# LongmaoTeamTf/deep_recommenders

Measured on AMD Instinct MI355X. Metric: examples/sec/node DeepFM (26 sparse feats, 10M vocab, dim 64), higher is better.
Workload: dtype f32; 1 GPU; DeepFM Criteo-shape synthetic training step (BASELINE.json configs[2]): 26 sparse + 13 dense, 10000000 vocab/field hashed on device, dim 64, DNN [256, 32]+[1] relu, sigmoid-CE, fused SGD; batch 65536 per GPU, ids uniform; tables on one GPU (66.6 GB); gemm_split=f16x2, global_batch=65536, parallelism=single, per_kernel_events=False

## Files before the change

deep_recommenders_amd/csrc/h2_occ.hip:

```cpp
#include "dr_common.h"
#include "rs_args.h"
#include <cstdlib>

namespace drrs {
namespace {

typedef _Float16 f16x4 __attribute__((ext_vector_type(4)));
typedef float f32x4 __attribute__((ext_vector_type(4)));
typedef float f32x16 __attribute__((ext_vector_type(16)));
typedef unsigned u32x4 __attribute__((ext_vector_type(4)));
typedef __attribute__((address_space(3))) void* lds_ptr_t;

#define OCC_DS_READ_B128(dst, addr, off) asm volatile("ds_read_b128 %0, %1 offset:%2" : "=v"(dst) : "v"(addr), "n"(off))
#define OCC_DS_WRITE_B64(addr, val, off) asm volatile("ds_write_b64 %0, %1 offset:%2" ::"v"(addr), "v"(val), "n"(off) : "memory")
#define OCC_DS_WRITE_B32(addr, val, off) asm volatile("ds_write_b32 %0, %1 offset:%2" ::"v"(addr), "v"(val), "n"(off) : "memory")

constexpr int BM = 256, BN = 256, BK = 32;
constexpr int PLANE = 256 * 64;
constexpr int A_OFF = 0, B_OFF = 2 * PLANE, STAGE = 4 * PLANE;

struct K4Args {
    const int32_t* ids_t;
    const uint8_t* flags;
    const int64_t* row_base; int32_t F;
    float* table; float* lin_w;
    const float* lin_old_t;
    const float* sum_x; const float* d_fm_logit;
    float scale;
    float* d_concat; int64_t ld_dc;
    uint32_t* table_amax;
};

template <int EPI, int DBG = 0>
__global__ __launch_bounds__(1024) void h2_occ_nt_kernel(RsArgs g, K4Args e) {
    __shared__ __attribute__((aligned(1024))) unsigned char smem[2 * STAGE + (EPI == 8 ? 10240 : 0)];

    const int tid = threadIdx.x, lane = tid & 63;
    const int wave = __builtin_amdgcn_readfirstlane(tid >> 6);
    const int l31 = lane & 31, hi = lane >> 5;
    const int wr = wave >> 2, wc = wave & 3;

    const int tiles_n = (g.N + BN - 1) / BN;
    const int tiles_m = (int)((g.M + BM - 1) / BM);
    const int ntiles = tiles_m * tiles_n;
    const int nk = (g.K + BK - 1) / BK;
    const bool ktail = (g.K % BK) != 0;
    const int kv4 = (g.K + 3) / 4 * 4;

    float s_a, inv_a, s_b, inv_b;
    h2_scale_of(g.a_amax[0], s_a, inv_a);
    h2_scale_of(g.b_amax[0], s_b, inv_b);
    const float h2_out = inv_a * inv_b;
    h2_mode_on();
    float cmax = 0.f;

    const unsigned lds0 = (unsigned)(uintptr_t)(lds_ptr_t)smem;
    const int sw = (l31 >> 2) & 3;
    const unsigned a_rd = lds0 + A_OFF + (64 * wr + l31) * 64 + (((2 * hi) ^ sw) << 4);
    const unsigned b_rd = lds0 + B_OFF + (64 * wc + l31) * 64 + (((2 * hi) ^ sw) << 4);
    const int r8 = lane >> 3, c4 = lane & 7;
    const int arow0 = 16 * wave + r8;
    const unsigned a_wr = lds0 + A_OFF + arow0 * 64 + ((((c4 >> 1) ^ ((arow0 >> 2) & 3)) << 4) | ((c4 & 1) << 3));
    const int avoff0 = (int)((arow0 * g.lda + 4 * c4) * 4), avoff1 = avoff0 + (int)(8 * g.lda * 4);
    const int brow = 16 * wave + (lane >> 2);
    const int bchunk = (lane & 3) ^ ((brow >> 2) & 3);
    const __amdgpu_buffer_rsrc_t brsrc = __builtin_amdgcn_make_buffer_rsrc(
        const_cast<__bf16*>(g.B), 0, (int)min((int64_t)0x7fffffff, 2 * g.b_ps * 2), 0x00020000);
    const int b_plane1 = (int)(g.b_ps * 2);

    f32x16 acc[2][2];
#pragma unroll
    for (int a = 0; a < 2; ++a)
#pragma unroll
        for (int b = 0; b < 2; ++b)
#pragma unroll
            for (int k = 0; k < 16; ++k) acc[a][b][k] = 0.f;

    for (int tile = blockIdx.x; tile < ntiles; tile += gridDim.x) {
        const int lid = xcd_remap(tile, ntiles);
        const int64_t tm0 = (int64_t)(lid / tiles_n) * BM;
        const int tn0 = (lid % tiles_n) * BN;
        const __amdgpu_buffer_rsrc_t arsrc = __builtin_amdgcn_make_buffer_rsrc(
            const_cast<float*>(g.A + tm0 * g.lda), 0, (int)min((int64_t)0x7fffffff, ((g.M - tm0 - 1) * g.lda + kv4) * 4), 0x00020000);
        const int bvoff = (int)(((int64_t)min(tn0 + brow, g.N - 1) * g.b_ld + bchunk * 8) * 2);
        auto issue_b = [&](int kt, int stage) {
            if constexpr (DBG & 1) { if (kt > 0) return; }
#pragma unroll
            for (int p = 0; p < 2; ++p) {
                unsigned char* dst = smem + stage * STAGE + B_OFF + p * PLANE + wave * 1024;
                __builtin_amdgcn_raw_ptr_buffer_load_lds(brsrc, (lds_ptr_t)dst, 16, bvoff, kt * (BK * 2) + p * b_plane1, 0, 0);
            }
        };
        f32x4 an0, an1;
        int an_kt = 0;
        auto load_a = [&](int kt) {
            if constexpr (DBG & 8) kt = 0;
            an_kt = kt;
            an0 = __builtin_bit_cast(f32x4, __builtin_amdgcn_raw_buffer_load_b128(arsrc, avoff0, kt * (BK * 4), 0));
            an1 = __builtin_bit_cast(f32x4, __builtin_amdgcn_raw_buffer_load_b128(arsrc, avoff1, kt * (BK * 4), 0));
        };
        auto wait_a = [&](bool) {};
        auto stage_a = [&](int which, int stage) {
            if constexpr (DBG & 64) return;
            f32x4 v = which == 0 ? an0 : an1;
            if (ktail) {
                const int k = an_kt * BK + 4 * c4;
                v[0] = k < g.K ? v[0] : 0.f; v[1] = k + 1 < g.K ? v[1] : 0.f; v[2] = k + 2 < g.K ? v[2] : 0.f; v[3] = k + 3 < g.K ? v[3] : 0.f;
            }
            f16x4 h, l;
            if constexpr (DBG & 256) {
                typedef float f32x2 __attribute__((ext_vector_type(2)));
                h = __builtin_bit_cast(f16x4, f32x2{v[0], v[1]});
                l = __builtin_bit_cast(f16x4, f32x2{v[2], v[3]});
            } else {
                const f32x4 x = v * s_a;
                h = __builtin_convertvector(x, f16x4);
                l = __builtin_convertvector(x - __builtin_convertvector(h, f32x4), f16x4);
            }
            const unsigned w = (which == 0 ? a_wr : (a_wr ^ 32u) + 512u) + stage * STAGE;
            if constexpr (DBG & 128) {
                asm volatile("" :: "v"(h), "v"(l), "v"(w));
            } else {
                OCC_DS_WRITE_B64(w, h, 0);
                OCC_DS_WRITE_B64(w, l, PLANE);
            }
        };
        f16x8 ah[2], al[2], bh[2], bl[2];
#define OCC_MMA(A, B)                                                                                       \
        _Pragma("unroll") for (int a = 0; a < 2; ++a)                                                       \
            _Pragma("unroll") for (int b = 0; b < 2; ++b)                                                   \
                if constexpr (!(DBG & 2)) acc[a][b] = __builtin_amdgcn_mfma_f32_32x32x16_f16(A[a], B[b], acc[a][b], 0, 0, 0);
#define OCC_MMA2(A, B, AI)                                                                                  \
        _Pragma("unroll") for (int b = 0; b < 2; ++b)                                                       \
            if constexpr (!(DBG & 2)) acc[AI][b] = __builtin_amdgcn_mfma_f32_32x32x16_f16(A[AI], B[b], acc[AI][b], 0, 0, 0);
#define OCC_RD(DST, ADDR, OFF) if constexpr (!(DBG & 32)) OCC_DS_READ_B128(DST, ADDR, OFF); else asm volatile("" : "=v"(DST));
#define OCC_FENCE() __builtin_amdgcn_sched_barrier(0)

        issue_b(0, 0);
        load_a(0);
        OCC_FENCE();
        wait_a(false);
        stage_a(0, 0);
        stage_a(1, 0);
        OCC_FENCE();
        load_a(nk > 1 ? 1 : 0);
        OCC_FENCE();
        asm volatile("s_waitcnt vmcnt(2) lgkmcnt(0)\n\ts_barrier" ::: "memory");
        if (nk > 1) issue_b(1, 1);
        {
            const unsigned aa = a_rd, bb = b_rd;
            OCC_RD(bl[0], bb, PLANE) OCC_RD(bl[1], bb, PLANE + 2048) OCC_RD(al[0], aa, PLANE) OCC_RD(al[1], aa, PLANE + 2048)
            OCC_RD(ah[0], aa, 0) OCC_RD(ah[1], aa, 2048) OCC_RD(bh[0], bb, 0) OCC_RD(bh[1], bb, 2048)
        }
        OCC_FENCE();

        for (int kt = 0; kt < nk; ++kt) {
            const int stage = kt & 1;
            const bool more = kt + 1 < nk;
            const unsigned aa1 = (a_rd + stage * STAGE) ^ 16u, bb1 = (b_rd + stage * STAGE) ^ 16u;
            if constexpr (!(DBG & 32)) asm volatile("s_waitcnt lgkmcnt(2)" : "+v"(ah[0]), "+v"(bl[0]), "+v"(ah[1]), "+v"(bl[1]), "+v"(al[0]), "+v"(al[1]));
            OCC_MMA(ah, bl)
            OCC_FENCE();
            OCC_RD(bl[0], bb1, PLANE) OCC_RD(bl[1], bb1, PLANE + 2048)
            if constexpr (!(DBG & 32)) asm volatile("s_waitcnt lgkmcnt(2)" : "+v"(bh[0]), "+v"(bh[1]));
            OCC_MMA2(al, bh, 0)
            OCC_FENCE();
            if (more) {
                wait_a(true);
                stage_a(0, stage ^ 1);
            }
            OCC_FENCE();
            OCC_MMA2(al, bh, 1)
            OCC_FENCE();
            OCC_RD(al[0], aa1, PLANE) OCC_RD(al[1], aa1, PLANE + 2048)
            OCC_MMA2(ah, bh, 0)
            OCC_FENCE();
            if (more) stage_a(1, stage ^ 1);
            OCC_FENCE();
            OCC_MMA2(ah, bh, 1)
            OCC_FENCE();
            OCC_RD(ah[0], aa1, 0) OCC_RD(ah[1], aa1, 2048) OCC_RD(bh[0], bb1, 0) OCC_RD(bh[1], bb1, 2048)
            load_a(kt + 2 < nk ? kt + 2 : nk - 1);
            OCC_FENCE();
            if constexpr (!(DBG & 32)) asm volatile("s_waitcnt lgkmcnt(2)" : "+v"(ah[0]), "+v"(ah[1]), "+v"(bl[0]), "+v"(bl[1]), "+v"(al[0]), "+v"(al[1]));
            OCC_MMA(ah, bl)
            OCC_FENCE();
            if constexpr (!(DBG & 512)) asm volatile("s_waitcnt vmcnt(2) lgkmcnt(0)\n\ts_barrier" : "+v"(bh[0]), "+v"(bh[1]) :: "memory");
            else asm volatile("s_waitcnt vmcnt(2) lgkmcnt(0)" : "+v"(bh[0]), "+v"(bh[1]) :: "memory");
            if (more) issue_b(kt + 2 < nk ? kt + 2 : nk - 1, stage);
            const unsigned aa2 = a_rd + (stage ^ 1) * STAGE, bb2 = b_rd + (stage ^ 1) * STAGE;
            if (more) { OCC_RD(bl[0], bb2, PLANE) OCC_RD(bl[1], bb2, PLANE + 2048) }
            OCC_FENCE();
            OCC_MMA(al, bh)
            OCC_FENCE();
            if (more) { OCC_RD(al[0], aa2, PLANE) OCC_RD(al[1], aa2, PLANE + 2048) }
            OCC_MMA(ah, bh)
            OCC_FENCE();
            if (more) { OCC_RD(ah[0], aa2, 0) OCC_RD(ah[1], aa2, 2048) OCC_RD(bh[0], bb2, 0) OCC_RD(bh[1], bb2, 2048) }
            OCC_FENCE();
            if constexpr (DBG & 2) acc[0][0][0] += (float)ah[0][0] + (float)ah[1][0] + (float)al[0][0] + (float)al[1][0] + (float)bh[0][0] + (float)bh[1][0] + (float)bl[0][0] + (float)bl[1][0];
        }
#undef OCC_MMA
#undef OCC_MMA2
#undef OCC_RD
#undef OCC_FENCE

        {
            const bool relu = g.act == 1;
            const bool interior = tm0 + BM <= g.M && tn0 + BN <= g.N;
            int lane_e = lane;
            asm volatile("" : "+v"(lane_e));
            const unsigned stg = lds0 + wave * 8192;
            const unsigned st_wr = stg + (4 * (lane_e >> 5)) * 256 + (lane_e & 31) * 4;
            const int prow = lane_e >> 4, pc4 = (lane_e & 15) * 4;
            const unsigned st_rd = stg + prow * 256 + pc4 * 4;
            const int col0 = tn0 + 64 * wc + pc4;
            float4 bj = make_float4(0.f, 0.f, 0.f, 0.f);
            if (g.bias != nullptr) {
                if (interior) bj = *reinterpret_cast<const float4*>(g.bias + col0);
                else {
                    bj.x = g.bias[min(col0, g.N - 1)]; bj.y = g.bias[min(col0 + 1, g.N - 1)];
                    bj.z = g.bias[min(col0 + 2, g.N - 1)]; bj.w = g.bias[min(col0 + 3, g.N - 1)];
                }
            }
            const int k4_f = (tn0 >> 6) + wc;
            const bool k4_on = EPI == 8 && k4_f < e.F;
            const int k4_rows = (int)min((int64_t)BM, g.M - tm0);
            const int k4_ldc4 = (int)(e.ld_dc * 4);
            __amdgpu_buffer_rsrc_t k4_t, k4_dl, k4_lo, k4_sx, k4_dc, k4_lw, k4_id, k4_fl;
            if constexpr (EPI == 8) {
                auto mk = [&](const void* p, int64_t bytes) {
                    const uint64_t b = reinterpret_cast<uint64_t>(p);
                    void* q = reinterpret_cast<void*>(((uint64_t)(unsigned)__builtin_amdgcn_readfirstlane((int)(b >> 32)) << 32) |
                                                      (unsigned)__builtin_amdgcn_readfirstlane((int)b));
                    return __builtin_amdgcn_make_buffer_rsrc(q, 0, (int)(unsigned)(bytes < 0xffffff00ll ? bytes : 0xffffff00ll), 0x00020000);
                };
                const int fc = k4_on ? k4_f : 0;
                const int64_t rb = e.row_base[fc];
                const bool has_lin = e.lin_w != nullptr;
                k4_t = mk(e.table + rb * 64, 0xffffff00ll);
                k4_dl = mk(e.d_fm_logit + tm0, (int64_t)k4_rows * 4);
                k4_lo = has_lin ? mk(e.lin_old_t + (int64_t)fc * g.M + tm0, (int64_t)k4_rows * 4) : k4_dl;
                k4_sx = mk(e.sum_x + tm0 * 64, (int64_t)k4_rows * 256);
                k4_dc = mk(e.d_concat + tm0 * e.ld_dc + 64 * fc, ((int64_t)k4_rows - 1) * e.ld_dc * 4 + 256);
                k4_lw = has_lin ? mk(e.lin_w + rb, 0x7fffffffll) : mk(e.table, 0);
                k4_id = mk(e.ids_t + (int64_t)fc * g.M + tm0, (int64_t)k4_rows * 4);
                k4_fl = mk(e.flags + tm0 * e.F, (int64_t)k4_rows * e.F);
            }
            if constexpr (EPI == 8) {
                constexpr unsigned SXP = 65536, DLP = 2 * STAGE, LOP = 2 * STAGE + 1024, UIP = 2 * STAGE + 1024 + 4096;
                const unsigned stq = lds0 + wave * 4096;
                const unsigned stq_wr = stq + (4 * (lane_e >> 5)) * 256 + (lane_e & 31) * 4;
                const unsigned stq_rd = stq + prow * 256 + pc4 * 4;
                {
#pragma unroll
                    for (int p4 = 0; p4 < 4; ++p4)
                        __builtin_amdgcn_raw_ptr_buffer_load_lds(k4_sx, (lds_ptr_t)(smem + SXP + (16 * wave + 4 * p4) * 256), 16,
                                                                 (16 * wave + 4 * p4 + (lane_e >> 4)) * 256 + (lane_e & 15) * 16, 0, 0, 0);
                    unsigned dlv = __builtin_amdgcn_raw_buffer_load_b32(k4_dl, (64 * wr + lane_e) * 4, 0, 0);
                    unsigned lov = __builtin_amdgcn_raw_buffer_load_b32(k4_lo, (64 * wr + lane_e) * 4, 0, 0);
                    int idl = (int)__builtin_amdgcn_raw_buffer_load_b32(k4_id, (64 * wr + lane_e) * 4, 0, 0);
                    int fll = (int)__builtin_amdgcn_raw_buffer_load_b8(k4_fl, (64 * wr + lane_e) * e.F + k4_f, 0, 0);
                    asm volatile("s_waitcnt vmcnt(0)" : "+v"(dlv), "+v"(lov), "+v"(idl), "+v"(fll) :: "memory");
                    const int uid = (k4_on && 64 * wr + lane_e < k4_rows && idl >= 0 && fll != 0) ? idl : -1;
                    OCC_DS_WRITE_B32(lds0 + DLP + (64 * wr + lane_e) * 4, dlv, 0);
                    OCC_DS_WRITE_B32(lds0 + LOP + wave * 256 + lane_e * 4, lov, 0);
                    OCC_DS_WRITE_B32(lds0 + UIP + wave * 256 + lane_e * 4, uid, 0);
                    asm volatile("s_waitcnt lgkmcnt(0)\n\ts_barrier" ::: "memory");
                }
                if (k4_on) {
#pragma unroll
                    for (int a = 0; a < 2; ++a) {
                        const int ml0 = 64 * wr + 32 * a + prow;
                        unsigned voff[8];
                        unsigned uqm = 0;
                        u32x4 t[8];
#pragma unroll
                        for (int it = 0; it < 8; ++it) {
                            const int uidv = *reinterpret_cast<const int*>(smem + UIP + wave * 256 + (32 * a + 4 * it + prow) * 4);
                            if (uidv >= 0) uqm |= 1u << it;
                            voff[it] = (unsigned)max(uidv, 0) * 256u + (unsigned)pc4 * 4u;
                            t[it] = __builtin_amdgcn_raw_buffer_load_b128(k4_t, (int)voff[it], 0, 2);
                        }
                        asm volatile("s_waitcnt vmcnt(0)" : "+v"(t[0]), "+v"(t[1]), "+v"(t[2]), "+v"(t[3]), "+v"(t[4]), "+v"(t[5]), "+v"(t[6]), "+v"(t[7]));
#pragma unroll
                        for (int q = 0; q < 2; ++q) {
#pragma unroll
                            for (int b = 0; b < 2; ++b)
#pragma unroll
                                for (int r8 = 0; r8 < 8; ++r8) {
                                    const int reg = 8 * q + r8;
                                    const float v = acc[a][b][reg] * h2_out;
                                    acc[a][b][reg] = 0.f;
                                    switch (b * 8 + r8) {
#define OCC_W(I) case I: OCC_DS_WRITE_B32(stq_wr, v, ((I & 3) + 8 * ((I & 7) >> 2)) * 256 + (I >> 3) * 128); break;
                                        OCC_W(0) OCC_W(1) OCC_W(2) OCC_W(3) OCC_W(4) OCC_W(5) OCC_W(6) OCC_W(7) OCC_W(8) OCC_W(9) OCC_W(10) OCC_W(11)
                                        OCC_W(12) OCC_W(13) OCC_W(14) OCC_W(15)
#undef OCC_W
                                    }
                                }
                            f32x4 v[4];
                            asm volatile("s_waitcnt lgkmcnt(0)\n\tds_read_b128 %0, %4 offset:0\n\tds_read_b128 %1, %4 offset:1024\n\t"
                                         "ds_read_b128 %2, %4 offset:2048\n\tds_read_b128 %3, %4 offset:3072\n\ts_waitcnt lgkmcnt(0)"
                                         : "=&v"(v[0]), "=&v"(v[1]), "=&v"(v[2]), "=&v"(v[3]) : "v"(stq_rd) : "memory");
#pragma unroll
                            for (int i = 0; i < 4; ++i) {
                                const int it = 4 * q + i;
                                const int ml = ml0 + 4 * it;
                                const bool uq = (uqm >> it) & 1u;
                                const f32x4 tv = __builtin_bit_cast(f32x4, t[it]);
                                const f32x4 sv = *reinterpret_cast<const f32x4*>(smem + SXP + ml * 256 + pc4 * 4);
                                const float dl = *reinterpret_cast<const float*>(smem + DLP + ml * 4);
                                const float lo = *reinterpret_cast<const float*>(smem + LOP + wave * 256 + (32 * a + 4 * it + prow) * 4);
                                float4 gq = make_float4(v[i][0], v[i][1], v[i][2], v[i][3]);
                                gq.x += dl * (sv[0] - tv[0]); gq.y += dl * (sv[1] - tv[1]);
                                gq.z += dl * (sv[2] - tv[2]); gq.w += dl * (sv[3] - tv[3]);
                                f32x4 r;
                                r[0] = fmaf(e.scale, gq.x, tv[0]); r[1] = fmaf(e.scale, gq.y, tv[1]);
                                r[2] = fmaf(e.scale, gq.z, tv[2]); r[3] = fmaf(e.scale, gq.w, tv[3]);
                                if (uq) cmax = fmaxf(cmax, fmaxf(fmaxf(fabsf(r[0]), fabsf(r[1])), fmaxf(fabsf(r[2]), fabsf(r[3]))));
                                __builtin_amdgcn_raw_buffer_store_b128(__builtin_bit_cast(u32x4, r), k4_t, uq ? (int)voff[it] : (int)0xffffff00u, 0, 2);
                                __builtin_amdgcn_raw_buffer_store_b128(__builtin_bit_cast(u32x4, v[i]), k4_dc,
                                                                       (uq || ml >= k4_rows) ? (int)0x80000000u : ml * k4_ldc4 + pc4 * 4, 0, 2);
                                __builtin_amdgcn_raw_buffer_store_b32(__builtin_bit_cast(unsigned, fmaf(e.scale, dl, lo)), k4_lw,
                                                                      (uq && pc4 == 0) ? (int)(voff[it] >> 6) : (int)0x80000000u, 0, 0);
                            }
                            asm volatile("s_waitcnt lgkmcnt(0)" ::: "memory");
                        }
                    }
                } else {
#pragma unroll
                    for (int a = 0; a < 2; ++a)
// ... 5 lines not shown
            } else
#pragma unroll
            for (int a = 0; a < 2; ++a) {
#pragma unroll
                for (int b = 0; b < 2; ++b)
#pragma unroll
                    for (int reg = 0; reg < 16; ++reg) {
                        const float v = acc[a][b][reg] * h2_out;
                        acc[a][b][reg] = 0.f;
                        switch (b * 16 + reg) {
#define OCC_W(I) case I: OCC_DS_WRITE_B32(st_wr, v, ((I & 3) + 8 * ((I & 15) >> 2)) * 256 + (I >> 4) * 128); break;
                            OCC_W(0) OCC_W(1) OCC_W(2) OCC_W(3) OCC_W(4) OCC_W(5) OCC_W(6) OCC_W(7) OCC_W(8) OCC_W(9) OCC_W(10) OCC_W(11)
                            OCC_W(12) OCC_W(13) OCC_W(14) OCC_W(15) OCC_W(16) OCC_W(17) OCC_W(18) OCC_W(19) OCC_W(20) OCC_W(21) OCC_W(22)
                            OCC_W(23) OCC_W(24) OCC_W(25) OCC_W(26) OCC_W(27) OCC_W(28) OCC_W(29) OCC_W(30) OCC_W(31)
#undef OCC_W
                        }
                    }
                asm volatile("s_waitcnt lgkmcnt(0)" ::: "memory");
                const int64_t rbase = tm0 + 64 * wr + 32 * a + prow;
#pragma unroll
                for (int half = 0; half < 2; ++half) {
                    f32x4 v[4];
                    float4 aux[4] = {};
#pragma unroll
                    for (int i = 0; i < 4; ++i) {
                        const int it = 4 * half + i;
                        switch (it) {
#define OCC_R(I) case I: OCC_DS_READ_B128(v[I & 3], st_rd, I * 1024); break;
                            OCC_R(0) OCC_R(1) OCC_R(2) OCC_R(3) OCC_R(4) OCC_R(5) OCC_R(6) OCC_R(7)
#undef OCC_R
                        }
                        if constexpr (EPI == 1 || EPI == 3) {
                            const int64_t row = rbase + 4 * it;
                            if (interior) {
                                aux[i] = EPI == 1 ? *reinterpret_cast<const float4*>(g.mask + row * g.ld_mask + col0)
                                                  : *reinterpret_cast<const float4*>(g.C + row * g.ldc + col0);
                            } else {
                                const float* src = EPI == 1 ? g.mask + min(row, g.M - 1) * g.ld_mask : g.C + min(row, g.M - 1) * g.ldc;
                                aux[i].x = src[min(col0, g.N - 1)]; aux[i].y = src[min(col0 + 1, g.N - 1)];
                                aux[i].z = src[min(col0 + 2, g.N - 1)]; aux[i].w = src[min(col0 + 3, g.N - 1)];
                            }
                        }
                    }
                    asm volatile("s_waitcnt lgkmcnt(0)" : "+v"(v[0]), "+v"(v[1]), "+v"(v[2]), "+v"(v[3]));
#pragma unroll
                    for (int i = 0; i < 4; ++i) {
                        const int64_t row = rbase + 4 * (4 * half + i);
                        float o[4] = {v[i][0] + bj.x, v[i][1] + bj.y, v[i][2] + bj.z, v[i][3] + bj.w};
                        const float ax[4] = {aux[i].x, aux[i].y, aux[i].z, aux[i].w};
#pragma unroll
                        for (int e = 0; e < 4; ++e) {
                            o[e] = relu ? fmaxf(o[e], 0.f) : o[e];
                            if constexpr (EPI == 1) o[e] = ax[e] > 0.f ? o[e] : 0.f;
                            if constexpr (EPI == 3) o[e] = ax[e] + o[e];
                        }
                        if (interior) {
#pragma unroll
                            for (int e = 0; e < 4; ++e) cmax = fmaxf(cmax, fabsf(o[e]));
                            *reinterpret_cast<float4*>(g.C + row * g.ldc + col0) = make_float4(o[0], o[1], o[2], o[3]);
                        } else if (row < g.M) {
#pragma unroll
                            for (int e = 0; e < 4; ++e)
                                if (col0 + e < g.N) {
                                    cmax = fmaxf(cmax, fabsf(o[e]));
                                    g.C[row * g.ldc + col0 + e] = o[e];
                                }
                        }
                    }
                }
                asm volatile("s_waitcnt lgkmcnt(0)" ::: "memory");
            }
            asm volatile("s_waitcnt vmcnt(0)\n\ts_barrier" ::: "memory");
        }
    }
    uint32_t* const amax_out = EPI == 8 ? e.table_amax : g.c_amax;
    if (amax_out != nullptr) {
        uint32_t m = __float_as_uint(cmax);
#pragma unroll
        for (int o = 32; o > 0; o >>= 1) m = max(m, (uint32_t)__shfl_xor((int)m, o, 64));
        if (lane == 0 && m > __hip_atomic_load(amax_out, __ATOMIC_RELAXED, __HIP_MEMORY_SCOPE_AGENT)) atomicMax(amax_out, m);
    }
}

}

int occ_nt_launch(const RsArgs& g, hipStream_t stream) {
    if (g.a_amax == nullptr || g.b_amax == nullptr) return 1;
    if (g.x0 != nullptr || g.tau != nullptr || g.pack_pos != nullptr || g.sm_part_m != nullptr || g.sm_lse != nullptr) return 1;
    if (g.mask == nullptr && !g.accumulate && g.K < 512) return 1;
    if ((g.ldc & 3) != 0 || (reinterpret_cast<uintptr_t>(g.C) & 15) != 0) return 1;
    if (g.mask != nullptr && ((g.ld_mask & 3) != 0 || (reinterpret_cast<uintptr_t>(g.mask) & 15) != 0)) return 1;
    if (g.bias != nullptr && (reinterpret_cast<uintptr_t>(g.bias) & 15) != 0) return 1;
    if (2 * g.b_ps * 2 + (int64_t)BK * 2 * ((g.K + BK - 1) / BK) > 0x7fffffffll) return 1;
    if ((int64_t)(BM + 8) * g.lda * 4 + (int64_t)g.K * 4 > 0x7fffffffll) return 1;
    const int64_t tiles = ((g.M + BM - 1) / BM) * ((g.N + BN - 1) / BN);
    if (tiles > 0x7fffffff) return DR_EINVAL;
    const int grid = (int)(tiles < 256 ? tiles : 256);
#ifdef DR_OCC_ABLATE
    {
        static const int dbg = [] { const char* e = getenv("DR_OCC_DBG"); return e ? atoi(e) : 0; }();
        if (dbg != 0 && g.mask == nullptr && !g.accumulate) {
#define OCC_ABL(D)                                                                                      \
            if (dbg == D) {                                                                             \
                hipLaunchKernelGGL((h2_occ_nt_kernel<0, D>), dim3(grid), dim3(1024), 0, stream, g, K4Args{});     \
                DR_CHECK_LAUNCH();                                                                      \
                return DR_OK;                                                                           \
            }
            OCC_ABL(2) OCC_ABL(32) OCC_ABL(34) OCC_ABL(1) OCC_ABL(8) OCC_ABL(9) OCC_ABL(64) OCC_ABL(73) OCC_ABL(137) OCC_ABL(265) OCC_ABL(393) OCC_ABL(521) OCC_ABL(585)
#undef OCC_ABL
        }
    }
#endif
    if (g.mask != nullptr) hipLaunchKernelGGL((h2_occ_nt_kernel<1>), dim3(grid), dim3(1024), 0, stream, g, K4Args{});
    else if (g.accumulate) hipLaunchKernelGGL((h2_occ_nt_kernel<3>), dim3(grid), dim3(1024), 0, stream, g, K4Args{});
    else hipLaunchKernelGGL((h2_occ_nt_kernel<0>), dim3(grid), dim3(1024), 0, stream, g, K4Args{});
    DR_CHECK_LAUNCH();
    return DR_OK;
}

}

extern "C" int dr_h2_dgrad_emb_sgd(const float* dy, int64_t ld_dy, const uint32_t* dy_amax, const void* w_planes, int64_t w_ps,
                                   int64_t w_ld, const uint32_t* w_amax, int64_t M, int32_t F, int32_t K, const int32_t* ids_t,
                                   const uint8_t* unique_flags, const int64_t* row_base, float* table, float* lin_w,
                                   const float* lin_old_t, const float* sum_x, const float* d_fm_logit, float scale, float* d_concat,
                                   int64_t ld_dconcat, uint32_t* table_amax, dr_stream_t stream) {
    using namespace drrs;
    if (M < 0 || F <= 0 || F > 64 || K <= 0 || !dy_amax || !w_amax) return DR_EINVAL;
    if (M == 0) return DR_OK;
    if (!dy || !w_planes || !ids_t || !unique_flags || !row_base || !table || !sum_x || !d_fm_logit || !d_concat) return DR_EINVAL;
    if ((lin_w != nullptr) != (lin_old_t != nullptr)) return DR_EINVAL;
    if ((reinterpret_cast<uintptr_t>(dy) & 15) != 0 || (ld_dy & 3) != 0 || ld_dy < K) return DR_EINVAL;
    if ((reinterpret_cast<uintptr_t>(w_planes) & 15) != 0 || w_ld < (K + BK - 1) / BK * BK || (w_ld & 7) != 0 || (w_ps & 7) != 0) return DR_EINVAL;
    if ((reinterpret_cast<uintptr_t>(d_concat) & 15) != 0 || (ld_dconcat & 3) != 0 || ld_dconcat < 64 * (int64_t)F) return DR_EINVAL;
    if ((reinterpret_cast<uintptr_t>(table) & 15) != 0 || (reinterpret_cast<uintptr_t>(sum_x) & 15) != 0) return DR_EINVAL;
    if (2 * w_ps * 2 + (int64_t)BK * 2 * ((K + BK - 1) / BK) > 0x7fffffffll) return DR_ESHAPE;
    if ((int64_t)(BM + 8) * ld_dy * 4 + (int64_t)K * 4 > 0x7fffffffll) return DR_ESHAPE;
    RsArgs g{};
    g.A = dy; g.lda = ld_dy; g.B = static_cast<const __bf16*>(w_planes); g.b_ps = w_ps; g.b_ld = w_ld;
    g.M = M; g.N = 64 * F; g.K = K;
    g.a_amax = dy_amax; g.b_amax = w_amax;
    K4Args e{ids_t, unique_flags, row_base, F, table, lin_w, lin_old_t, sum_x, d_fm_logit, scale, d_concat, ld_dconcat, table_amax};
    const int64_t tiles = ((M + BM - 1) / BM) * ((g.N + BN - 1) / BN);
    if (tiles > 0x7fffffff) return DR_EINVAL;
    const int grid = (int)(tiles < 256 ? tiles : 256);
    hipLaunchKernelGGL((h2_occ_nt_kernel<8>), dim3(grid), dim3(1024), 0, dr_s(stream), g, e);
    DR_CHECK_LAUNCH();
    return DR_OK;
}
```

deep_recommenders_amd/engine.py:

```python
import math
from typing import List, Optional, Sequence

import torch

from . import ops


_SIDE_STREAMS = {}


def _side_streams(device):
    key = str(torch.device(device))
    if key not in _SIDE_STREAMS:
        _SIDE_STREAMS[key] = (torch.cuda.Stream(device=device), torch.cuda.Stream(device=device))
    return _SIDE_STREAMS[key]


def _pad4(n):
    return (n + 3) // 4 * 4


def _os_env(name, default):
    import os
    return os.environ.get(name, default)
# ... 482 lines not shown
        if head and self.fuse_tail and self._in_train_step:
            W1, W2 = self.Ws[-2], self.Ws[-1]
            adam = self.optimizer == "adam"
            def tail(parts, x=x, W1=W1, W2=W2):
                return ops.tower_tail_fused(
                    x, W1, self.bs[-2], W2, self.bs[-1], self.fm_logit, labels, loss_mode, 1.0 if adam else -self.lr, self.dhs[nl - 3],
                    dst_W1=self.gWs[-2] if adam else "inplace", dst_b1=self.gbs[-2] if adam else "inplace",
                    dst_W2=self.gWs[-1] if adam else "inplace", dst_b2=self.gbs[-1] if adam else "inplace",
                    prob=self.prob, d_logit=self.d_logit, d_h=self.dhs[-1], loss=self.loss, workspace=self.tail_ws, parts=parts,
                    dx_amax=self.dh0_amax if (self.h2 and nl - 2 == 1 and (parts & 1)) else None)
            work = 4.0 * B * (2 * W1.shape[0] + W1.shape[1] + 4)
            if self.reduce_side:
                self._k("tower_tail_fused", "hbm", work, lambda: tail(1))
                self._side_part2(lambda: tail(2))
            else:
                self._k("tower_tail_fused", "hbm", work, lambda: tail(3))
            self._tail_done = True
            return self.prob
        if head:
            W1, W2 = self.Ws[-2], self.Ws[-1]
            def head(parts, x=x, W1=W1, W2=W2):
                return ops.tower_head_fwd_bwd(
                    x, W1, self.bs[-2], W2, self.bs[-1], self.fm_logit, labels, loss_mode,
                    1.0 if self.optimizer == "adam" else -self.lr, act=1,
                    prob=self.prob, d_logit=self.d_logit, d_h=self.dhs[-1], loss=self.loss, workspace=self.head_ws,
                    dst_W2=self.gWs[-1] if self.optimizer == "adam" else "inplace",
                    dst_b2=self.gbs[-1] if self.optimizer == "adam" else "inplace", parts=parts)
            if self.reduce_side and self._in_train_step:
                self._k("tower_head_fwd_bwd", "hbm", 4.0 * B * (W1.shape[0] + W1.shape[1] + 4), lambda: head(1))
                self._side_part2(lambda: head(2))
            else:
                self._k("tower_head_fwd_bwd", "hbm", 4.0 * B * (W1.shape[0] + W1.shape[1] + 4), lambda: head(3))
            return self.prob
        if labels is None:
            labels = self.prob
        ops.bce_fwd_bwd(self.fm_logit, labels, loss_mode, workspace=self.ws, logits_b=self.hs[-1],
                        out=(self.prob, self.d_logit, self.loss))
        return self.prob

    def backward_and_update(self):
        F, D, lr = self.F, self.D, self.lr
        adam = self.optimizer == "adam"
        lin_side = self.lin_side and not adam and not self.sort_inline
        if lin_side:
            self.ev_dlogit.record()
            with torch.cuda.stream(self.side):
                self.side.wait_event(self.ev_dlogit)
                self._k("emb_lin_update_unique(side stream, overlapped)", "overlap", self.B * self.F * 16,
                        lambda: ops.emb_lin_update_unique(self.ids, self.row_base, self.plan, self.d_logit, -lr, self.lin_w))
                self.ev_lin.record(self.side)
        sc = 1.0 if adam else -lr
        n = len(self.Ws)
        dy = self.d_logit.reshape(-1, 1)
        top = n - 1
        if self._head_done:
            top = n - 2
            dy = self.dhs[-1]
        if self._tail_done:
            top = n - 3
            dy = self.dhs[n - 3]
        for i in range(top, -1, -1):
            x = self.concat[:, :self.in_dim] if i == 0 else self.hs[i - 1]
            W = self.Ws[i]
            dstW, dstb = (self.gWs[i], self.gbs[i]) if adam else (W, self.bs[i])
            fl = 2.0 * self.B * W.shape[0] * W.shape[1]
            if i > 0:
                dx = self.dhs[i - 1]
                rs = self.hs[i - 1] if self.acts[i - 1] else None
            else:
                dx = self.d_concat[:, :self.in_dim]
                rs = None
            if i > 0 and self.fuse_narrow and self.narrow_ws[i] is not None:
                def narrow(parts, x=x, dy=dy, W=W, dx=dx, i=i, dstW=dstW, dstb=dstb):
                    return ops.linear_bwd_narrow(x, dy, W, sc, dstW, dstb, dx, relu_mask=True, workspace=self.narrow_ws[i], parts=parts,
                                                 dx_amax=self.dh0_amax if (i == 1 and self.h2 and (parts & 1)) else None)
                if self.reduce_side and self._in_train_step:
                    self._k("linear_bwd_narrow_L%d" % i, "hbm", 4.0 * self.B * (2 * W.shape[0] + W.shape[1]), lambda: narrow(1))
                    self._side_part2(lambda: narrow(2))
                else:
                    self._k("linear_bwd_narrow_L%d" % i, "hbm", 4.0 * self.B * (2 * W.shape[0] + W.shape[1]), lambda: narrow(3))
                dy = dx
                continue
            if i == 0 and self.fuse_k4 and self._lin_old_valid and not adam and not self.overlap_dw:
                self._backward_l0_fused_k4(x, dy, sc, dstW, dstb, fl)
                dy = None
                continue
            if i == 0 and self.h2:
                if not (n > 1 and self.fuse_narrow and self.narrow_ws[1] is not None):
                    ops.h2_amax(dy, self.dh0_amax)
                self._k("linear_bwd_dx_L%d" % i, "mfma", fl,
                        lambda dy=dy, rs=rs, dx=dx, i=i: ops.h2_linear_nt(dy, self.dh0_amax, self.wplanes[i].w, mask=rs, out=dx))
            elif self.wplanes[i] is not None:
                self._k("linear_bwd_dx_L%d" % i, "mfma", fl,
                        lambda dy=dy, rs=rs, dx=dx, i=i: ops.bf3_linear_nt(dy, self.wplanes[i].w, mask=rs, out=dx))
            else:
                self._k("linear_bwd_dx_L%d" % i, "mfma", fl,
                        lambda dy=dy, W=W, rs=rs, dx=dx: ops.linear_bwd_dx(dy, W, relu_src=rs, out=dx))
            if i == 0 and self.sorted_bwd and self._plan_prefetched and self.lean_events:
                torch.cuda.current_stream().wait_event(self.ev_sorted)
            if i == 0 and self.overlap_dw:
                self.ev_dx.record()
                with torch.cuda.stream(self.side2):
                    self.side2.wait_event(self.ev_dx)
                    self._k("linear_bwd_dw_L%d" % i, "mfma", fl,
                            lambda x=x, dy=dy, i=i, dstW=dstW, dstb=dstb: self._wgrad(i, x, dy, sc, dstW, dstb))
                    if self.wplanes[i] is not None and not adam:
                        self.wplanes[i].refresh()
                    self.ev_dw.record(self.side2)
                dy = dx
                continue
            self._k("linear_bwd_dw_L%d" % i, "mfma", fl,
                    lambda x=x, dy=dy, i=i, dstW=dstW, dstb=dstb: self._wgrad(i, x, dy, sc, dstW, dstb))
            if self.wplanes[i] is not None and not adam:
                if self.sorted_bwd and not self.sort_inline:
                    self.ev_dw_done.record()
                    self._refresh_stream = self.side
                    with torch.cuda.stream(self.side):
                        self.side.wait_event(self.ev_dw_done)
                        if self._wgrad_reduce_deferred(i) and self.h2:
                            ops.h2_wgrad_emb(self._ids_t[self.cur], self.row_base, self.table, self.tab_amax, self.dense_pad, self.dense_amax,
                                             dy, self.dh0_amax, sc, dstW, dstb, workspace=self.wg_ws[0], parts=2)
                        elif self._wgrad_reduce_deferred(i):
                            ops.bf3_wgrad_emb(self._ids_t[self.cur], self.row_base, self.table, self.dense_pad, dy, sc, dstW, dstb,
                                              workspace=self.wg_ws[0], parts=2)
                        self.wplanes[i].refresh()
                        self.ev_planes.record(self.side)
                    self._planes_pending = True
                    self._planes_pending_l0 = (i == 0)
                else:
                    self.wplanes[i].refresh()
            dy = dx
        if adam:
            self._adam_finish()
        elif self._k4_fused_done:
            self._k4_fused_done = False
        elif self.sorted_bwd:
            if not (self._plan_prefetched and self.lean_events):
                torch.cuda.current_stream().wait_event(self.ev_sorted)
            if self.no_concat and not self._k4_det:
                ops.emb_snapshot_sorted_rows(self.plan, self.table, self.R, self.x_sorted)
            mark = self._prefetch_mark()
            k4 = lambda parts: ops.emb_pool_bwd_sorted(self.ids, self.row_base, self.plan, D, self.R, self.d_concat, self.d_logit,
                                                       -lr, self.table, self.lin_w, self.lin_bias,
                                                       concat=None if self.no_concat else self.concat, sum_x=self.sum_x,
                                                       x_sorted=self.x_sorted if self.no_concat else None, parts=parts,
                                                       lin_old_t=self.lin_old_t if (self._lin_old_valid and not lin_side) else None,
                                                       table_amax=self.tab_amax if (self.h2 and not self._exp_no_k4_amax) else None)
            sk = 4 if lin_side else 0
            self._k("emb_pool_bwd", "hbm", self.alg_bytes_bwd() - (self.B * self.F * 8 if lin_side else 0),
                    lambda: k4(1 | sk))
            if self.no_concat:
                self._k("emb_hot_rows_apply", "hbm", 0, lambda: k4(2 | sk))
            if lin_side:
                torch.cuda.current_stream().wait_event(self.ev_lin)
            self._prefetch_issue(mark)
        else:
            self._k("emb_pool_bwd", "hbm", self.alg_bytes_bwd(),
                    lambda: ops.emb_pool_bwd(self.ids, F, self.col_start, self.row_base, D, self.d_concat, self.concat,
                                             self.sum_x, self.d_logit, -lr, self.table, self.lin_w, self.lin_bias))
        if self._small_pending:
            torch.cuda.current_stream().wait_event(self.ev_small)
            self._small_pending = False
        if self.overlap_dw and not adam:
            torch.cuda.current_stream().wait_event(self.ev_dw)

    def _backward_l0_fused_k4(self, x, dy, sc, dstW, dstb, fl):
# ... 121 lines not shown
```

Before: 66.15 million examples/sec.

## Add ping-pong fused layer-0 backward kernel overlapping GEMM with embedding epilogue

Adds a new kernel in which two 8-wave groups in a 1024-thread block alternate between the GEMM main loop and the fused embedding-update epilogue on 128-row tiles. The two groups stay in lockstep through a matched barrier count, so one group's MFMA work can hide the other's gather and scatter memory latency. It is enabled by default behind an env toggle, and the older kernel gains debug ablation modes. The engine also computes the dy amax before the fused path, which adds a small kernel but may fix a scaling input that was missing. The risks are barrier-count mismatches, halved M-tile reuse of B, and higher LDS use.

```diff
diff --git a/deep_recommenders_amd/csrc/h2_occ.hip b/deep_recommenders_amd/csrc/h2_occ.hip
--- a/deep_recommenders_amd/csrc/h2_occ.hip
+++ b/deep_recommenders_amd/csrc/h2_occ.hip
@@ -1,5 +1,6 @@
 #include "dr_common.h"
 #include "rs_args.h"
+#include <algorithm>
 #include <cstdlib>
 
 namespace drrs {
@@ -136,6 +137,7 @@
 #define OCC_RD(DST, ADDR, OFF) if constexpr (!(DBG & 32)) OCC_DS_READ_B128(DST, ADDR, OFF); else asm volatile("" : "=v"(DST));
 #define OCC_FENCE() __builtin_amdgcn_sched_barrier(0)
 
+        if constexpr (!(DBG & 2048)) {
         issue_b(0, 0);
         load_a(0);
         OCC_FENCE();
@@ -199,6 +201,7 @@
             if (more) { OCC_RD(ah[0], aa2, 0) OCC_RD(ah[1], aa2, 2048) OCC_RD(bh[0], bb2, 0) OCC_RD(bh[1], bb2, 2048) }
             OCC_FENCE();
             if constexpr (DBG & 2) acc[0][0][0] += (float)ah[0][0] + (float)ah[1][0] + (float)al[0][0] + (float)al[1][0] + (float)bh[0][0] + (float)bh[1][0] + (float)bl[0][0] + (float)bl[1][0];
+        }
         }
 #undef OCC_MMA
 #undef OCC_MMA2
@@ -247,7 +250,14 @@
                 k4_id = mk(e.ids_t + (int64_t)fc * g.M + tm0, (int64_t)k4_rows * 4);
                 k4_fl = mk(e.flags + tm0 * e.F, (int64_t)k4_rows * e.F);
             }
-            if constexpr (EPI == 8) {
+            if constexpr (EPI == 8 && (DBG & 1024)) {
+#pragma unroll
+                for (int a = 0; a < 2; ++a)
+#pragma unroll
+                    for (int b = 0; b < 2; ++b)
+#pragma unroll
+                        for (int reg = 0; reg < 16; ++reg) cmax = fmaxf(cmax, fabsf(acc[a][b][reg])), acc[a][b][reg] = 0.f;
+            } else if constexpr (EPI == 8) {
                 constexpr unsigned SXP = 65536, DLP = 2 * STAGE, LOP = 2 * STAGE + 1024, UIP = 2 * STAGE + 1024 + 4096;
                 const unsigned stq = lds0 + wave * 4096;
                 const unsigned stq_wr = stq + (4 * (lane_e >> 5)) * 256 + (lane_e & 31) * 4;
@@ -419,6 +429,323 @@
     }
 }
 
+
+constexpr int PM = 128;
+constexpr int PA_PLANE = PM * 64, PB_PLANE = BN * 64;
+constexpr int PA_OFF = 0, PB_OFF = 2 * PA_PLANE, PSTAGE = 2 * PA_PLANE + 2 * PB_PLANE;
+constexpr int P_SXP = 2 * PSTAGE;
+constexpr int P_STQ = P_SXP + PM * 256;
+constexpr int P_DLP = P_STQ + 8 * 2048;
+constexpr int P_LOP = P_DLP + PM * 4;
+constexpr int P_UIP = P_LOP + 8 * 256;
+constexpr int P_LDS = P_UIP + 8 * 256;
+constexpr int P_EPI_BARRIERS = 7;
+
+__global__ __launch_bounds__(1024) void h2_occ_pp_kernel(RsArgs g, K4Args e) {
+    __shared__ __attribute__((aligned(1024))) unsigned char smem[P_LDS];
+
+    const int tid = threadIdx.x, lane = tid & 63;
+    const int wave = __builtin_amdgcn_readfirstlane(tid >> 6);
+    const int grp = wave >> 3, wg = wave & 7;
+    const int wr = wg >> 2, wc = wg & 3;
+
+    const int tiles_n = (g.N + BN - 1) / BN;
+    const int tiles_m = (int)((g.M + PM - 1) / PM);
+    const int ntiles = tiles_m * tiles_n;
+    const int nk = (g.K + BK - 1) / BK;
+    const bool ktail = (g.K % BK) != 0;
+    const int kv4 = (g.K + 3) / 4 * 4;
+    const int nb = max(nk + 1, P_EPI_BARRIERS);
+
+    float s_a, inv_a, s_b, inv_b;
+    h2_scale_of(g.a_amax[0], s_a, inv_a);
+    h2_scale_of(g.b_amax[0], s_b, inv_b);
+    const float h2_out = inv_a * inv_b;
+    h2_mode_on();
+    float cmax = 0.f;
+
+    const unsigned lds0 = (unsigned)(uintptr_t)(lds_ptr_t)smem;
+    const __amdgpu_buffer_rsrc_t brsrc = __builtin_amdgcn_make_buffer_rsrc(
+        const_cast<__bf16*>(g.B), 0, (int)min((int64_t)0x7fffffff, 2 * g.b_ps * 2), 0x00020000);
+    const int b_plane1 = (int)(g.b_ps * 2);
+
+    f32x16 acc[2][2];
+#pragma unroll
+    for (int a = 0; a < 2; ++a)
+#pragma unroll
+        for (int b = 0; b < 2; ++b)
+#pragma unroll
+            for (int k = 0; k < 16; ++k) acc[a][b][k] = 0.f;
+
+    auto bar = [] { asm volatile("s_barrier" ::: "memory"); };
+    auto tile_of = [&](int i, int64_t& tm0, int& tn0) __attribute__((always_inline)) {
+        const int lid = xcd_remap((int)blockIdx.x + i * (int)gridDim.x, ntiles);
+        tm0 = (int64_t)(lid / tiles_n) * PM;
+        tn0 = (lid % tiles_n) * BN;
+    };
+
+    auto main_loop = [&](int i) __attribute__((always_inline)) {
+        int64_t tm0; int tn0;
+        tile_of(i, tm0, tn0);
+        int lane_m = lane;
+        asm volatile("" : "+v"(lane_m));
+        const int l31 = lane_m & 31, hi = lane_m >> 5;
+        const int sw = (l31 >> 2) & 3;
+        const unsigned a_rd = lds0 + PA_OFF + (64 * wr + l31) * 64 + (((2 * hi) ^ sw) << 4);
+        const unsigned b_rd = lds0 + PB_OFF + (64 * wc + l31) * 64 + (((2 * hi) ^ sw) << 4);
+        const int r8 = lane_m >> 3, c4 = lane_m & 7;
+        const int arow0 = 16 * wg + r8;
+        const unsigned a_wr = lds0 + PA_OFF + arow0 * 64 + ((((c4 >> 1) ^ ((arow0 >> 2) & 3)) << 4) | ((c4 & 1) << 3));
+        const int avoff0 = (int)((arow0 * g.lda + 4 * c4) * 4), avoff1 = avoff0 + (int)(8 * g.lda * 4);
+        const int brow = 16 * wg + (lane_m >> 2);
+        const int bchunk = (lane_m & 3) ^ ((brow >> 2) & 3);
+        const __amdgpu_buffer_rsrc_t arsrc = __builtin_amdgcn_make_buffer_rsrc(
+            const_cast<float*>(g.A + tm0 * g.lda), 0, (int)min((int64_t)0x7fffffff, ((g.M - tm0 - 1) * g.lda + kv4) * 4), 0x00020000);
+        const int bvoff0 = (int)(((int64_t)min(tn0 + brow, g.N - 1) * g.b_ld + bchunk * 8) * 2);
+        const int bvoff1 = (int)(((int64_t)min(tn0 + brow + 128, g.N - 1) * g.b_ld + bchunk * 8) * 2);
+        auto issue_b = [&](int kt, int stage) __attribute__((always_inline)) {
+#pragma unroll
+            for (int p = 0; p < 2; ++p) {
+                unsigned char* dst = smem + stage * PSTAGE + PB_OFF + p * PB_PLANE + wg * 1024;
+                __builtin_amdgcn_raw_ptr_buffer_load_lds(brsrc, (lds_ptr_t)dst, 16, bvoff0, kt * (BK * 2) + p * b_plane1, 0, 0);
+                __builtin_amdgcn_raw_ptr_buffer_load_lds(brsrc, (lds_ptr_t)(dst + 128 * 64), 16, bvoff1, kt * (BK * 2) + p * b_plane1, 0, 0);
+            }
+        };
+        f32x4 an0, an1;
+        int an_kt = 0;
+        auto load_a = [&](int kt) __attribute__((always_inline)) {
+            an_kt = kt;
+            an0 = __builtin_bit_cast(f32x4, __builtin_amdgcn_raw_buffer_load_b128(arsrc, avoff0, kt * (BK * 4), 0));
+            an1 = __builtin_bit_cast(f32x4, __builtin_amdgcn_raw_buffer_load_b128(arsrc, avoff1, kt * (BK * 4), 0));
+        };
+        auto stage_a = [&](int which, int stage) __attribute__((always_inline)) {
+            f32x4 v = which == 0 ? an0 : an1;
+            if (ktail) {
+                const int k = an_kt * BK + 4 * c4;
+                v[0] = k < g.K ? v[0] : 0.f; v[1] = k + 1 < g.K ? v[1] : 0.f; v[2] = k + 2 < g.K ? v[2] : 0.f; v[3] = k + 3 < g.K ? v[3] : 0.f;
+            }
+            const f32x4 x = v * s_a;
+            const f16x4 h = __builtin_convertvector(x, f16x4);
+            const f16x4 l = __builtin_convertvector(x - __builtin_convertvector(h, f32x4), f16x4);
+            const unsigned w = (which == 0 ? a_wr : (a_wr ^ 32u) + 512u) + stage * PSTAGE;
+            OCC_DS_WRITE_B64(w, h, 0);
+            OCC_DS_WRITE_B64(w, l, PA_PLANE);
+        };
+        f16x8 ah[2], al[2], bh[2], bl[2];
+#define PP_MMA(A, B)                                                                                        \
+        _Pragma("unroll") for (int a = 0; a < 2; ++a)                                                       \
+            _Pragma("unroll") for (int b = 0; b < 2; ++b)                                                   \
+                acc[a][b] = __builtin_amdgcn_mfma_f32_32x32x16_f16(A[a], B[b], acc[a][b], 0, 0, 0);
+#define PP_MMA2(A, B, AI)                                                                                   \
+        _Pragma("unroll") for (int b = 0; b < 2; ++b)                                                       \
+            acc[AI][b] = __builtin_amdgcn_mfma_f32_32x32x16_f16(A[AI], B[b], acc[AI][b], 0, 0, 0);
+#define PP_RD(DST, ADDR, OFF) OCC_DS_READ_B128(DST, ADDR, OFF);
+#define PP_FENCE() __builtin_amdgcn_sched_barrier(0)
+        issue_b(0, 0);
+        load_a(0);
+        PP_FENCE();
+        stage_a(0, 0);
+        stage_a(1, 0);
+        PP_FENCE();
+        load_a(nk > 1 ? 1 : 0);
+        PP_FENCE();
+        asm volatile("s_waitcnt vmcnt(2) lgkmcnt(0)\n\ts_barrier" ::: "memory");
+        if (nk > 1) issue_b(1, 1);
+        {
+            const unsigned aa = a_rd, bb = b_rd;
+            PP_RD(bl[0], bb, PB_PLANE) PP_RD(bl[1], bb, PB_PLANE + 2048) PP_RD(al[0], aa, PA_PLANE) PP_RD(al[1], aa, PA_PLANE + 2048)
+            PP_RD(ah[0], aa, 0) PP_RD(ah[1], aa, 2048) PP_RD(bh[0], bb, 0) PP_RD(bh[1], bb, 2048)
+        }
+        PP_FENCE();
+        for (int kt = 0; kt < nk; ++kt) {
+            const int stage = kt & 1;
+            const bool more = kt + 1 < nk;
+            const unsigned aa1 = (a_rd + stage * PSTAGE) ^ 16u, bb1 = (b_rd + stage * PSTAGE) ^ 16u;
+            asm volatile("s_waitcnt lgkmcnt(2)" : "+v"(ah[0]), "+v"(bl[0]), "+v"(ah[1]), "+v"(bl[1]), "+v"(al[0]), "+v"(al[1]));
+            PP_MMA(ah, bl)
+            PP_FENCE();
+            PP_RD(bl[0], bb1, PB_PLANE) PP_RD(bl[1], bb1, PB_PLANE + 2048)
+            asm volatile("s_waitcnt lgkmcnt(2)" : "+v"(bh[0]), "+v"(bh[1]));
+            PP_MMA2(al, bh, 0)
+            PP_FENCE();
+            if (more) stage_a(0, stage ^ 1);
+            PP_FENCE();
+            PP_MMA2(al, bh, 1)
+            PP_FENCE();
+            PP_RD(al[0], aa1, PA_PLANE) PP_RD(al[1], aa1, PA_PLANE + 2048)
+            PP_MMA2(ah, bh, 0)
+            PP_FENCE();
+            if (more) stage_a(1, stage ^ 1);
+            PP_FENCE();
+            PP_MMA2(ah, bh, 1)
+            PP_FENCE();
+            PP_RD(ah[0], aa1, 0) PP_RD(ah[1], aa1, 2048) PP_RD(bh[0], bb1, 0) PP_RD(bh[1], bb1, 2048)
+            load_a(kt + 2 < nk ? kt + 2 : nk - 1);
+            PP_FENCE();
+            asm volatile("s_waitcnt lgkmcnt(2)" : "+v"(ah[0]), "+v"(ah[1]), "+v"(bl[0]), "+v"(bl[1]), "+v"(al[0]), "+v"(al[1]));
+            PP_MMA(ah, bl)
+            PP_FENCE();
+            asm volatile("s_waitcnt vmcnt(2) lgkmcnt(0)\n\ts_barrier" : "+v"(bh[0]), "+v"(bh[1]) :: "memory");
+            if (more) issue_b(kt + 2 < nk ? kt + 2 : nk - 1, stage);
+            const unsigned aa2 = a_rd + (stage ^ 1) * PSTAGE, bb2 = b_rd + (stage ^ 1) * PSTAGE;
+            if (more) { PP_RD(bl[0], bb2, PB_PLANE) PP_RD(bl[1], bb2, PB_PLANE + 2048) }
+            PP_FENCE();
+            PP_MMA(al, bh)
+            PP_FENCE();
+            if (more) { PP_RD(al[0], aa2, PA_PLANE) PP_RD(al[1], aa2, PA_PLANE + 2048) }
+            PP_MMA(ah, bh)
+            PP_FENCE();
+            if (more) { PP_RD(ah[0], aa2, 0) PP_RD(ah[1], aa2, 2048) PP_RD(bh[0], bb2, 0) PP_RD(bh[1], bb2, 2048) }
+            PP_FENCE();
+        }
+#undef PP_MMA
+#undef PP_MMA2
+#undef PP_RD
+#undef PP_FENCE
+        for (int b = nk + 1; b < nb; ++b) bar();
+    };
+
+    auto epilogue = [&](int i) __attribute__((always_inline)) {
+        int64_t tm0; int tn0;
+        tile_of(i, tm0, tn0);
+        int lane_e = lane;
+        asm volatile("" : "+v"(lane_e));
+        const int prow = lane_e >> 4, pc4 = (lane_e & 15) * 4;
+        const int k4_f = (tn0 >> 6) + wc;
+        const bool k4_on = k4_f < e.F;
+        const int k4_rows = (int)min((int64_t)PM, g.M - tm0);
+        const int k4_ldc4 = (int)(e.ld_dc * 4);
+        auto mk = [&](const void* p, int64_t bytes) __attribute__((always_inline)) {
+            const uint64_t b = reinterpret_cast<uint64_t>(p);
+            void* q = reinterpret_cast<void*>(((uint64_t)(unsigned)__builtin_amdgcn_readfirstlane((int)(b >> 32)) << 32) |
+                                              (unsigned)__builtin_amdgcn_readfirstlane((int)b));
+            return __builtin_amdgcn_make_buffer_rsrc(q, 0, (int)(unsigned)(bytes < 0xffffff00ll ? bytes : 0xffffff00ll), 0x00020000);
+        };
+        const int fc = k4_on ? k4_f : 0;
+        const int64_t rb = e.row_base[fc];
+        const bool has_lin = e.lin_w != nullptr;
+        const __amdgpu_buffer_rsrc_t k4_t = mk(e.table + rb * 64, 0xffffff00ll);
+        const __amdgpu_buffer_rsrc_t k4_dl = mk(e.d_fm_logit + tm0, (int64_t)k4_rows * 4);
+        const __amdgpu_buffer_rsrc_t k4_lo = has_lin ? mk(e.lin_old_t + (int64_t)fc * g.M + tm0, (int64_t)k4_rows * 4) : k4_dl;
+        const __amdgpu_buffer_rsrc_t k4_sx = mk(e.sum_x + tm0 * 64, (int64_t)k4_rows * 256);
+        const __amdgpu_buffer_rsrc_t k4_dc = mk(e.d_concat + tm0 * e.ld_dc + 64 * fc, ((int64_t)k4_rows - 1) * e.ld_dc * 4 + 256);
+        const __amdgpu_buffer_rsrc_t k4_lw = has_lin ? mk(e.lin_w + rb, 0x7fffffffll) : mk(e.table, 0);
+        const __amdgpu_buffer_rsrc_t k4_id = mk(e.ids_t + (int64_t)fc * g.M + tm0, (int64_t)k4_rows * 4);
+        const __amdgpu_buffer_rsrc_t k4_fl = mk(e.flags + tm0 * e.F, (int64_t)k4_rows * e.F);
+        const unsigned stq = lds0 + P_STQ + wg * 2048;
+        const unsigned stq_wr = stq + (4 * (lane_e >> 5)) * 256 + (lane_e & 31) * 4;
+        const unsigned stq_rd = stq + prow * 256 + pc4 * 4;
+
+#pragma unroll
+        for (int p4 = 0; p4 < 4; ++p4)
+            __builtin_amdgcn_raw_ptr_buffer_load_lds(k4_sx, (lds_ptr_t)(smem + P_SXP + (16 * wg + 4 * p4) * 256), 16,
+                                                     (16 * wg + 4 * p4 + (lane_e >> 4)) * 256 + (lane_e & 15) * 16, 0, 0, 0);
+        unsigned dlv = __builtin_amdgcn_raw_buffer_load_b32(k4_dl, (64 * wr + lane_e) * 4, 0, 0);
+        unsigned lov = __builtin_amdgcn_raw_buffer_load_b32(k4_lo, (64 * wr + lane_e) * 4, 0, 0);
+        int idl = (int)__builtin_amdgcn_raw_buffer_load_b32(k4_id, (64 * wr + lane_e) * 4, 0, 0);
+        int fll = (int)__builtin_amdgcn_raw_buffer_load_b8(k4_fl, (64 * wr + lane_e) * e.F + k4_f, 0, 0);
+        bar();
+        asm volatile("s_waitcnt vmcnt(0)" : "+v"(dlv), "+v"(lov), "+v"(idl), "+v"(fll) :: "memory");
+        const int uid = (k4_on && 64 * wr + lane_e < k4_rows && idl >= 0 && fll != 0) ? idl : -1;
+        OCC_DS_WRITE_B32(lds0 + P_DLP + (64 * wr + lane_e) * 4, dlv, 0);
+        OCC_DS_WRITE_B32(lds0 + P_LOP + wg * 256 + lane_e * 4, lov, 0);
+        OCC_DS_WRITE_B32(lds0 + P_UIP + wg * 256 + lane_e * 4, uid, 0);
+        asm volatile("s_waitcnt lgkmcnt(0)" ::: "memory");
+        auto uid_of = [&](int a, int it) __attribute__((always_inline)) {
+            return *reinterpret_cast<const int*>(smem + P_UIP + wg * 256 + (32 * a + 4 * it + prow) * 4);
+        };
+        u32x4 t[8];
+        auto issue_rows = [&](int a) __attribute__((always_inline)) {
+#pragma unroll
+            for (int it = 0; it < 8; ++it)
+                t[it] = __builtin_amdgcn_raw_buffer_load_b128(k4_t, (int)((unsigned)max(uid_of(a, it), 0) * 256u + (unsigned)pc4 * 4u), 0, 2);
+        };
+        auto eighth = [&](int a, int h) __attribute__((always_inline)) {
+            const int ml0 = 64 * wr + 32 * a + prow;
+#pragma unroll
+            for (int b = 0; b < 2; ++b)
+#pragma unroll
+                for (int r = 0; r < 4; ++r) {
+                    const int reg = 4 * h + r;
+                    const float v = acc[a][b][reg] * h2_out;
+                    acc[a][b][reg] = 0.f;
+                    switch (b * 4 + r) {
+#define PP_W(I) case I: OCC_DS_WRITE_B32(stq_wr, v, (I & 3) * 256 + (I >> 2) * 128); break;
+                        PP_W(0) PP_W(1) PP_W(2) PP_W(3) PP_W(4) PP_W(5) PP_W(6) PP_W(7)
+#undef PP_W
+                    }
+                }
+            f32x4 v[2];
+            asm volatile("s_waitcnt lgkmcnt(0)\n\tds_read_b128 %0, %2 offset:0\n\tds_read_b128 %1, %2 offset:1024\n\ts_waitcnt lgkmcnt(0)"
+                         : "=&v"(v[0]), "=&v"(v[1]) : "v"(stq_rd) : "memory");
+#pragma unroll
+            for (int i = 0; i < 2; ++i) {
+                const int it = 2 * h + i;
+                const int ml = ml0 + 4 * it;
+                const int uidv = uid_of(a, it);
+                const bool uq = uidv >= 0;
+                const unsigned voff = (unsigned)uidv * 256u + (unsigned)pc4 * 4u;
+                const f32x4 tv = __builtin_bit_cast(f32x4, t[it]);
+                const f32x4 sv = *reinterpret_cast<const f32x4*>(smem + P_SXP + ml * 256 + pc4 * 4);
+                const float dl = *reinterpret_cast<const float*>(smem + P_DLP + ml * 4);
+                const float lo = *reinterpret_cast<const float*>(smem + P_LOP + wg * 256 + (32 * a + 4 * it + prow) * 4);
+                float4 gq = make_float4(v[i][0], v[i][1], v[i][2], v[i][3]);
+                gq.x += dl * (sv[0] - tv[0]); gq.y += dl * (sv[1] - tv[1]);
+                gq.z += dl * (sv[2] - tv[2]); gq.w += dl * (sv[3] - tv[3]);
+                f32x4 r;
+                r[0] = fmaf(e.scale, gq.x, tv[0]); r[1] = fmaf(e.scale, gq.y, tv[1]);
+                r[2] = fmaf(e.scale, gq.z, tv[2]); r[3] = fmaf(e.scale, gq.w, tv[3]);
+                if (uq) cmax = fmaxf(cmax, fmaxf(fmaxf(fabsf(r[0]), fabsf(r[1])), fmaxf(fabsf(r[2]), fabsf(r[3]))));
+                __builtin_amdgcn_raw_buffer_store_b128(__builtin_bit_cast(u32x4, r), k4_t, uq ? (int)voff : (int)0xffffff00u, 0, 2);
+                __builtin_amdgcn_raw_buffer_store_b128(__builtin_bit_cast(u32x4, v[i]), k4_dc,
+                                                       (uq || ml >= k4_rows) ? (int)0x80000000u : ml * k4_ldc4 + pc4 * 4, 0, 2);
+                __builtin_amdgcn_raw_buffer_store_b32(__builtin_bit_cast(unsigned, fmaf(e.scale, dl, lo)), k4_lw,
+                                                      (uq && pc4 == 0) ? (int)(voff >> 6) : (int)0x80000000u, 0, 0);
+            }
+            asm volatile("s_waitcnt lgkmcnt(0)" ::: "memory");
+        };
+        auto wait_rows = [&]() __attribute__((always_inline)) {
+            asm volatile("s_waitcnt vmcnt(0)" : "+v"(t[0]), "+v"(t[1]), "+v"(t[2]), "+v"(t[3]), "+v"(t[4]), "+v"(t[5]), "+v"(t[6]), "+v"(t[7]));
+        };
+        if (k4_on) issue_rows(0);
+        bar();
+        if (k4_on) { wait_rows(); eighth(0, 0); eighth(0, 1); }
+        bar();
+        if (k4_on) { eighth(0, 2); eighth(0, 3); issue_rows(1); }
+        bar();
+        if (k4_on) { wait_rows(); eighth(1, 0); eighth(1, 1); }
+        bar();
+        if (k4_on) { eighth(1, 2); eighth(1, 3); }
+        else {
+#pragma unroll
+            for (int a = 0; a < 2; ++a)
+#pragma unroll
+                for (int b = 0; b < 2; ++b)
+#pragma unroll
+                    for (int reg = 0; reg < 16; ++reg) acc[a][b][reg] = 0.f;
+        }
+        bar();
+        asm volatile("s_waitcnt vmcnt(0)" ::: "memory");
+        bar();
+        for (int b = P_EPI_BARRIERS; b < nb; ++b) bar();
+    };
+
+    const int n = (int)blockIdx.x < ntiles ? (ntiles - 1 - (int)blockIdx.x) / (int)gridDim.x + 1 : 0;
+    auto idle = [&]() __attribute__((always_inline)) { for (int b = 0; b < nb; ++b) bar(); };
+    if (grp == 1) idle();
+    for (int i = grp; i < n; i += 2) {
+        main_loop(i);
+        epilogue(i);
+    }
+    if (((n ^ grp) & 1) == 0) idle();
+    if (e.table_amax != nullptr) {
+        uint32_t m = __float_as_uint(cmax);
+#pragma unroll
+        for (int o = 32; o > 0; o >>= 1) m = max(m, (uint32_t)__shfl_xor((int)m, o, 64));
+        if (lane == 0 && m > __hip_atomic_load(e.table_amax, __ATOMIC_RELAXED, __HIP_MEMORY_SCOPE_AGENT)) atomicMax(e.table_amax, m);
+    }
+}
+
 }
 
 int occ_nt_launch(const RsArgs& g, hipStream_t stream) {
@@ -478,10 +805,24 @@
     g.M = M; g.N = 64 * F; g.K = K;
     g.a_amax = dy_amax; g.b_amax = w_amax;
     K4Args e{ids_t, unique_flags, row_base, F, table, lin_w, lin_old_t, sum_x, d_fm_logit, scale, d_concat, ld_dconcat, table_amax};
-    const int64_t tiles = ((M + BM - 1) / BM) * ((g.N + BN - 1) / BN);
+    static const bool overlap = [] { const char* v = getenv("DR_FUSED_K4_OVERLAP"); return !(v && v[0] == '0' && v[1] == 0); }();
+    const int64_t tiles = ((M + (overlap ? PM : BM) - 1) / (overlap ? PM : BM)) * ((g.N + BN - 1) / BN);
     if (tiles > 0x7fffffff) return DR_EINVAL;
     const int grid = (int)(tiles < 256 ? tiles : 256);
-    hipLaunchKernelGGL((h2_occ_nt_kernel<8>), dim3(grid), dim3(1024), 0, dr_s(stream), g, e);
+#ifdef DR_OCC_ABLATE
+    {
+        static const int dbg = [] { const char* v = getenv("DR_OCC_DBG"); return v ? atoi(v) : 0; }();
+        if (dbg == 1024 || dbg == 2048) {
+            const int grid8 = (int)std::min<int64_t>(((M + BM - 1) / BM) * ((g.N + BN - 1) / BN), 256);
+            if (dbg == 1024) hipLaunchKernelGGL((h2_occ_nt_kernel<8, 1024>), dim3(grid8), dim3(1024), 0, dr_s(stream), g, e);
+            else hipLaunchKernelGGL((h2_occ_nt_kernel<8, 2048>), dim3(grid8), dim3(1024), 0, dr_s(stream), g, e);
+            DR_CHECK_LAUNCH();
+            return DR_OK;
+        }
+    }
+#endif
+    if (overlap) hipLaunchKernelGGL(h2_occ_pp_kernel, dim3(grid), dim3(1024), 0, dr_s(stream), g, e);
+    else hipLaunchKernelGGL((h2_occ_nt_kernel<8>), dim3(grid), dim3(1024), 0, dr_s(stream), g, e);
     DR_CHECK_LAUNCH();
     return DR_OK;
 }
diff --git a/deep_recommenders_amd/engine.py b/deep_recommenders_amd/engine.py
--- a/deep_recommenders_amd/engine.py
+++ b/deep_recommenders_amd/engine.py
@@ -588,6 +588,8 @@
                 dy = dx
                 continue
             if i == 0 and self.fuse_k4 and self._lin_old_valid and not adam and not self.overlap_dw:
+                if self.h2 and not (n > 1 and self.fuse_narrow and self.narrow_ws[1] is not None):
+                    ops.h2_amax(dy, self.dh0_amax)
                 self._backward_l0_fused_k4(x, dy, sc, dstW, dstb, fl)
                 dy = None
                 continue
```

Result: faster. 68.21 million examples/sec, median of 6 (+3.1%).
